# davenza/PyBNesian

Hardware: AMD Instinct MI355X
Metric: KDE slogl M-samples/s (higher is better)
Workload: dtype f64; 1 GPU; C2: ProductKDE.slogl f64, N_train=1000000, N_test=100000 per GPU, d=8, normal-reference diagonal bandwidth; parallelism=test rows sharded over 1 GPU(s), training set replicated, ranks=1

## Files before the change

### pybnesian_amd/csrc/capi.hip

```cpp
#include <algorithm>
#include <cmath>
#include <cstdlib>
#include <cstring>
#include <memory>
#include <numeric>

#include "common.hpp"
#include "hostmath.hpp"
#include "kde_kernels.hpp"
#include "kde_model.hpp"
#include "kde_handle.hpp"
#include "stats_kernels.hpp"

namespace pbn {
static thread_local std::string g_last_error;
void set_last_error(const std::string& s) { g_last_error = s; }
std::recursive_mutex& api_mutex() {
    static std::recursive_mutex m;
    return m;
}
}

using namespace pbn;

extern "C" {

const char* pbn_last_error(void) { return g_last_error.c_str(); }
const char* pbn_version(void) { return "pbn_hip 0.1 (gfx950)"; }

int pbn_ctx_create(int device, pbn_ctx** out) {
    return guarded([&] {
        if (!out) throw invalid_error("pbn_ctx_create: out is null");
        int count = 0;
        HIP_CHECK(hipGetDeviceCount(&count));
        if (device < 0 || device >= count) throw device_error("pbn_ctx_create: no such HIP device");
        HIP_CHECK(hipSetDevice(device));
        auto ctx = std::make_unique<pbn_ctx>();
        ctx->device = device;
        HIP_CHECK(hipStreamCreateWithFlags(&ctx->stream, hipStreamNonBlocking));
        hipDeviceProp_t prop;
        HIP_CHECK(hipGetDeviceProperties(&prop, device));
        ctx->num_cus = prop.multiProcessorCount > 0 ? prop.multiProcessorCount : 256;
        *out = ctx.release();
    });
}

}

void pbn::ctx_release(pbn_ctx* ctx) {
    if (ctx->refs.fetch_sub(1, std::memory_order_acq_rel) != 1) return;
    PBN_API_LOCK;
    (void)hipSetDevice(ctx->device);
    (void)hipStreamSynchronize(ctx->stream);
    ctx->scratch_part.release();
    ctx->scratch_q.release();
    ctx->scratch_misc.release();
    ctx->scratch_red.release();
    (void)hipStreamDestroy(ctx->stream);
    for (auto& ln : ctx->parked)
        if (ln.stream) { (void)hipStreamSynchronize(ln.stream); (void)hipStreamDestroy(ln.stream); (void)hipEventDestroy(ln.fence); }
    delete ctx;
}

extern "C" {

void pbn_ctx_destroy(pbn_ctx* ctx) {
    if (ctx) pbn::ctx_release(ctx);
}

int pbn_ctx_sync(pbn_ctx* ctx) {
    return guarded(mu_of(ctx), [&] {
        HIP_CHECK(hipSetDevice(ctx->device));
        HIP_CHECK(hipStreamSynchronize(ctx->stream));
    });
}

void* pbn_ctx_stream(pbn_ctx* ctx) { return (void*)ctx->stream; }

static void drain_timers(pbn_ctx* ctx) {
    HIP_CHECK(hipStreamSynchronize(ctx->stream));
    for (auto& t : ctx->pending) {
        float ms = 0.f;
        if (hipEventElapsedTime(&ms, t.e0, t.e1) == hipSuccess) {
            ctx->kernel_ms[t.which] += ms;
            ctx->kernel_launches[t.which] += 1;
        }
        (void)hipEventDestroy(t.e0);
        (void)hipEventDestroy(t.e1);
    }
    ctx->pending.clear();
}

int pbn_ctx_set_profiling(pbn_ctx* ctx, int on) {
    return guarded(mu_of(ctx), [&] {
        if (!ctx) throw invalid_error("pbn_ctx_set_profiling: null context");
        HIP_CHECK(hipSetDevice(ctx->device));
        drain_timers(ctx);
        ctx->profiling = on == 1;
        ctx->timing = on == 2;
        for (int i = 0; i < PBN_NUM_KERNEL_CLASSES; ++i) { ctx->kernel_ms[i] = 0; ctx->kernel_launches[i] = 0; }
    });
}

int pbn_ctx_kernel_time(pbn_ctx* ctx, int kernel_class, double* total_ms, int64_t* launches) {
    return guarded(mu_of(ctx), [&] {
        if (!ctx || kernel_class < 0 || kernel_class >= PBN_NUM_KERNEL_CLASSES) throw invalid_error("pbn_ctx_kernel_time: bad argument");
        HIP_CHECK(hipSetDevice(ctx->device));
        drain_timers(ctx);
        if (total_ms) *total_ms = ctx->kernel_ms[kernel_class];
        if (launches) *launches = ctx->kernel_launches[kernel_class];
    });
}

// ... 295 lines not shown
            k->cA.alloc((size_t)m.ntiles * k->cdf_KS * 64 * sizeof(double));
            k->cN.alloc((size_t)m.ntiles * 16 * sizeof(double));
            k->cU.alloc((size_t)m.ntiles * 16 * sizeof(double));
            pbn::WidePackArgs wa{};
            fill_cdf_pack_wide(ctx, wa, *k, train, cols);
            wa.rows = nullptr; wa.row0 = row0; wa.n0 = n; wa.row1 = 0; wa.n = n; wa.ntiles = m.ntiles; wa.is_query = 0;
            wa.pack = (double*)k->cA.p; wa.npack = (double*)k->cN.p; wa.upack = (double*)k->cU.p;
            KernelTimer kt(ctx, PBN_K_PACK);
            launch_pack_wide(wa, ctx->stream);
        }
    }
    *out = k.release();
}

int pbn_kde_fit(pbn_ctx* ctx, const pbn_table* train, const int* cols, int d, int64_t row0, int64_t n,
                const double* bandwidth, int kind, const double* center, pbn_kde** out) {
    return guarded(mu_of(ctx), [&] {
        if (kind != PBN_BW_FULL && kind != PBN_BW_DIAG) throw invalid_error("pbn_kde_fit: unknown bandwidth kind");
        kde_fit_impl(ctx, train, cols, d, row0, n, bandwidth, kind, false, center, out);
    });
}

int pbn_ckde_fit(pbn_ctx* ctx, const pbn_table* train, const int* cols, int d, int64_t row0, int64_t n,
                 const double* H, const double* center, pbn_kde** out) {
    return guarded(mu_of(ctx), [&] { kde_fit_impl(ctx, train, cols, d, row0, n, H, PBN_BW_FULL, true, center, out, true); });
}

void pbn_kde_destroy(pbn_kde* k) {
    if (!k) return;
    pbn::ctx_pin pin_(k->ctx);
    std::lock_guard<std::recursive_mutex> lock_(mu_of(k));
    (void)hipSetDevice(k->ctx->device);
    (void)hipStreamSynchronize(k->ctx->stream);
    delete k;
}

int64_t pbn_kde_num_instances(const pbn_kde* k) { return k ? k->m.N : 0; }
double pbn_kde_lognorm(const pbn_kde* k, int which) { return which ? k->m.lognorm_marg : k->m.lognorm; }

static void kde_eval_enqueue(pbn_kde* k, const pbn_table* test, const int* cols, int64_t row0, int64_t n,
                             double* dev_logl, double* dev_sum, bool precise = false) {
    if (!k) throw invalid_error("KDE factor not fitted.");
    if (k->split_joint) {
        pbn_ctx* ctx = k->ctx;
        check_cols(test, cols, k->m.d, "pbn_kde_logl");
        const size_t per = dev_logl ? (size_t)std::max<int64_t>(n, 1) : 0;
        ctx->scratch_split.reserve(2 * per + 2);
        double* lj = dev_logl ? ctx->scratch_split.p : nullptr;
        double* lm = dev_logl ? ctx->scratch_split.p + per : nullptr;
        double* sj = dev_sum ? ctx->scratch_split.p + 2 * per : nullptr;
        double* sm = dev_sum ? sj + 1 : nullptr;
        const bool lanes = pbn::score_lanes() > 1 && !ctx->profiling;
        if (lanes) { ctx->ensure_lanes(1); ctx->lanes_wait_for_stream(1); }
        pbn::kde_eval_enqueue(ctx, k->split_joint->m, test, cols, row0, n, lj, sj, nullptr, nullptr, precise);
        {
            pbn::LaneSwitch lane(ctx, lanes ? 1 : 0);
            pbn::kde_eval_enqueue(ctx, k->split_marg->m, test, cols + 1, row0, n, lm, sm, nullptr, nullptr, precise);
        }
        if (lanes) ctx->stream_waits_for_lane(0);
        if (dev_logl) launch_diff(dev_logl, lj, lm, n, ctx->stream);
        if (dev_sum) launch_diff(dev_sum, sj, sm, 1, ctx->stream);
        return;
    }
    pbn::kde_eval_enqueue(k->ctx, k->m, test, cols, row0, n, dev_logl, dev_sum, nullptr, nullptr, precise);
}

int pbn_kde_logl_dev(pbn_kde* k, const pbn_table* test, const int* cols, int64_t row0, int64_t n, double* dev_out) {
    return guarded(mu_of(k), [&] {
        if (!dev_out && n > 0) throw invalid_error("pbn_kde_logl_dev: null output");
        kde_eval_enqueue(k, test, cols, row0, n, dev_out, nullptr);
    });
}

int pbn_kde_logl(pbn_kde* k, const pbn_table* test, const int* cols, int64_t row0, int64_t n, double* out) {
    return guarded(mu_of(k), [&] {
        if (!out && n > 0) throw invalid_error("pbn_kde_logl: null output");
        if (!k) throw invalid_error("KDE factor not fitted.");
        dev_buf<double> tmp((size_t)std::max<int64_t>(n, 1));
        kde_eval_enqueue(k, test, cols, row0, n, tmp.p, nullptr);
        if (n > 0) HIP_CHECK(hipMemcpyAsync(out, tmp.p, (size_t)n * sizeof(double), hipMemcpyDeviceToHost, k->ctx->stream));
        HIP_CHECK(hipStreamSynchronize(k->ctx->stream));
    });
}

int pbn_ckde_cdf(pbn_kde* k, const pbn_table* test, const int* cols, int64_t row0, int64_t n, double* out) {
    return guarded(mu_of(k), [&] {
        if (!k) throw invalid_error("CKDE factor not fitted.");
        if (!k->ckde) throw invalid_error("pbn_ckde_cdf: the handle was not created by pbn_ckde_fit");
        if (!out && n > 0) throw invalid_error("pbn_ckde_cdf: null output");
        pbn_ctx* ctx = k->ctx;
        const KdeModel& m = k->m;
        check_cols(test, cols, m.d, "pbn_ckde_cdf");
        check_range(test, row0, n, "pbn_ckde_cdf");
        if (test->dtype != m.dtype) throw invalid_error("Data type of training and test datasets is different.");
        if (test->ctx->device != ctx->device) throw invalid_error("pbn_ckde_cdf: test table lives on another device");
        HIP_CHECK(hipSetDevice(ctx->device));
        if (n == 0) return;
        const int fdt = k->cdf_wide ? PBN_F64 : m.dtype;
        const size_t es = dtype_size(fdt);
        const int64_t nqtiles = ceil_div(n, 16);
        const size_t b_b = (size_t)nqtiles * k->cdf_KS * 64 * es, n_b = (size_t)nqtiles * 16 * es;
        ctx->scratch_q.reserve(b_b + 2 * n_b + 256);
        char* q = ctx->scratch_q.p;
        struct { void* pack; void* npack; void* upack; } pa{q, q + b_b, q + b_b + n_b};
        if (k->cdf_wide) {
            pbn::WidePackArgs wq{};
            fill_cdf_pack_wide(ctx, wq, *k, test, cols);
            wq.rows = nullptr; wq.row0 = row0; wq.n0 = n; wq.row1 = 0; wq.n = n; wq.ntiles = nqtiles; wq.is_query = 1;
            wq.pack = (double*)pa.pack; wq.npack = (double*)pa.npack; wq.upack = (double*)pa.upack;
            KernelTimer kt(ctx, PBN_K_PACK);
            launch_pack_wide(wq, ctx->stream);
        } else {
            PackArgs pq{};
            fill_cdf_pack(pq, *k, test, cols);
            pq.row0 = row0; pq.n0 = n; pq.row1 = 0; pq.n = n; pq.ntiles = nqtiles; pq.is_query = 1;
            pq.pack = pa.pack; pq.npack = pa.npack; pq.upack = pa.upack;
            KernelTimer kt(ctx, PBN_K_PACK);
// ... 47 lines not shown
```

### pybnesian_amd/csrc/common.hpp

```cpp
#pragma once
#include <hip/hip_runtime.h>
#include <cstdlib>
#include <utility>

#include <cstdarg>
#include <cstdint>
#include <cstdio>
#include <atomic>
#include <mutex>
#include <stdexcept>
#include <string>
#include <vector>

#include "../../include/pbn_hip.h"

#define PBN_MAX_D_HOST 33

namespace pbn {

struct invalid_error : std::runtime_error {
    using std::runtime_error::runtime_error;
};
struct singular_error : std::runtime_error {
    using std::runtime_error::runtime_error;
};
struct device_error : std::runtime_error {
    using std::runtime_error::runtime_error;
};

void set_last_error(const std::string& s);

std::recursive_mutex& api_mutex();
#define PBN_API_LOCK std::lock_guard<std::recursive_mutex> pbn_api_lock_(::pbn::api_mutex())

inline void hip_check(hipError_t e, const char* what, const char* file, int line) {
    if (e != hipSuccess) {
        char buf[512];
        snprintf(buf, sizeof buf, "HIP error %d (%s) in %s at %s:%d", (int)e, hipGetErrorString(e), what, file, line);
        throw device_error(buf);
    }
}
#define HIP_CHECK(x) ::pbn::hip_check((x), #x, __FILE__, __LINE__)

template <typename F>
int guarded(std::recursive_mutex& mu, F&& f) noexcept {
    try {
        std::lock_guard<std::recursive_mutex> lock(mu);
        f();
        return PBN_OK;
    } catch (const invalid_error& e) {
        set_last_error(e.what());
        return PBN_ERR_INVALID;
    } catch (const singular_error& e) {
        set_last_error(e.what());
        return PBN_ERR_SINGULAR;
    } catch (const device_error& e) {
        set_last_error(e.what());
        return PBN_ERR_DEVICE;
    } catch (const std::bad_alloc&) {
        set_last_error("out of host memory");
        return PBN_ERR_DEVICE;
    } catch (const std::exception& e) {
        set_last_error(e.what());
        return PBN_ERR_INVALID;
    }
}
template <typename F>
int guarded(F&& f) noexcept {
    return guarded(api_mutex(), std::forward<F>(f));
}

template <typename T>
struct dev_buf {
    T* p = nullptr;
    size_t n = 0;
    dev_buf() = default;
    explicit dev_buf(size_t count) { alloc(count); }
    dev_buf(const dev_buf&) = delete;
    dev_buf& operator=(const dev_buf&) = delete;
    dev_buf(dev_buf&& o) noexcept : p(o.p), n(o.n) { o.p = nullptr; o.n = 0; }
    dev_buf& operator=(dev_buf&& o) noexcept {
        if (this != &o) {
            release();
            p = o.p; n = o.n; o.p = nullptr; o.n = 0;
        }
        return *this;
    }
    ~dev_buf() { release(); }
    void alloc(size_t count) {
        release();
        n = count;
        if (count) HIP_CHECK(hipMalloc((void**)&p, count * sizeof(T)));
    }
    void reserve(size_t count) {
        if (count > n) alloc(count);
    }
    void release() {
        if (p) (void)hipFree(p);
        p = nullptr; n = 0;
    }
};

inline size_t dtype_size(int dtype) { return dtype == PBN_F32 ? 4 : 8; }

inline int64_t ceil_div(int64_t a, int64_t b) { return (a + b - 1) / b; }

}


struct pbn_ctx {
    std::recursive_mutex mu;
    std::atomic<int> refs{1};
    int device = 0;
    hipStream_t stream = nullptr;
    int num_cus = 256;
    pbn::dev_buf<char> scratch_part;
    pbn::dev_buf<char> scratch_q;
    pbn::dev_buf<char> scratch_misc;
    pbn::dev_buf<double> scratch_red;
    pbn::dev_buf<char> scratch_train;
    pbn::dev_buf<char> scratch_prune;
    pbn::dev_buf<char> scratch_pruneq;
    pbn::dev_buf<char> scratch_sort;
    pbn::dev_buf<double> scratch_split;
    pbn::dev_buf<double> scratch_w;
    pbn::dev_buf<char> scratch_group;
    pbn::dev_buf<double> scratch_sums;
    std::vector<std::vector<char>> staged;
    void drop_staged() { staged.clear(); }
    struct Lane {
        hipStream_t stream = nullptr;
        pbn::dev_buf<char> part, q, misc, train, prune, pruneq, sort, group;
        pbn::dev_buf<double> red, split, w;
        hipEvent_t fence = nullptr;
    };
    static constexpr int MAX_PARKED = 3;
    Lane parked[MAX_PARKED];
    void ensure_lanes(int n_parked) {
        for (int k = 0; k < n_parked && k < MAX_PARKED; ++k)
            if (!parked[k].stream) {
                HIP_CHECK(hipStreamCreateWithFlags(&parked[k].stream, hipStreamNonBlocking));
                HIP_CHECK(hipEventCreateWithFlags(&parked[k].fence, hipEventDisableTiming));
            }
    }
    void swap_lane(int k) {
        Lane& alt = parked[k];
        std::swap(stream, alt.stream);
        std::swap(scratch_part, alt.part); std::swap(scratch_q, alt.q); std::swap(scratch_misc, alt.misc);
        std::swap(scratch_train, alt.train); std::swap(scratch_prune, alt.prune); std::swap(scratch_pruneq, alt.pruneq);
        std::swap(scratch_sort, alt.sort); std::swap(scratch_group, alt.group); std::swap(scratch_red, alt.red); std::swap(scratch_split, alt.split); std::swap(scratch_w, alt.w);
    }
    void lanes_wait_for_stream(int n_parked) {
        for (int k = 0; k < n_parked && k < MAX_PARKED; ++k) {
            HIP_CHECK(hipEventRecord(parked[k].fence, stream));
            HIP_CHECK(hipStreamWaitEvent(parked[k].stream, parked[k].fence, 0));
        }
    }
    void stream_waits_for_lane(int k) {
        HIP_CHECK(hipEventRecord(parked[k].fence, parked[k].stream));
        HIP_CHECK(hipStreamWaitEvent(stream, parked[k].fence, 0));
    }
    void sync_lanes(int n_parked) {
        for (int k = 0; k < n_parked && k < MAX_PARKED; ++k)
            if (parked[k].stream) HIP_CHECK(hipStreamSynchronize(parked[k].stream));
    }
    bool profiling = false;
    bool timing = false;
    struct Timed { hipEvent_t e0, e1; int which; };
    std::vector<Timed> pending;
    double kernel_ms[PBN_NUM_KERNEL_CLASSES] = {0};
    int64_t kernel_launches[PBN_NUM_KERNEL_CLASSES] = {0};
};

namespace pbn {
void ctx_release(pbn_ctx* c);
inline void ctx_retain(pbn_ctx* c) { c->refs.fetch_add(1, std::memory_order_relaxed); }
struct ctx_ptr {
    pbn_ctx* p = nullptr;
    ctx_ptr() = default;
    ctx_ptr(const ctx_ptr&) = delete;
    ctx_ptr& operator=(const ctx_ptr&) = delete;
    ctx_ptr& operator=(pbn_ctx* c) {
        if (c) ctx_retain(c);
        if (p) ctx_release(p);
        p = c;
        return *this;
    }
    ~ctx_ptr() { if (p) ctx_release(p); }
    operator pbn_ctx*() const { return p; }
    pbn_ctx* operator->() const { return p; }
};
struct ctx_pin {
    pbn_ctx* c;
    explicit ctx_pin(pbn_ctx* c_) : c(c_) { if (c) ctx_retain(c); }
    ~ctx_pin() { if (c) ctx_release(c); }
    ctx_pin(const ctx_pin&) = delete;
    ctx_pin& operator=(const ctx_pin&) = delete;
};
}

namespace pbn {
inline std::recursive_mutex& mu_of(const pbn_ctx* c) { return c ? const_cast<pbn_ctx*>(c)->mu : api_mutex(); }
template <typename H>
inline std::recursive_mutex& mu_of(const H* h) { return h ? mu_of(static_cast<const pbn_ctx*>(h->ctx)) : api_mutex(); }
}

namespace pbn {
inline long long knob_ll(const char* name, long long dflt) { const char* e = std::getenv(name); return (e && *e) ? std::atoll(e) : dflt; }
inline int knob_int(const char* name, int dflt) { return (int)knob_ll(name, dflt); }
inline double knob_double(const char* name, double dflt) { const char* e = std::getenv(name); return (e && *e) ? std::atof(e) : dflt; }
}
#ifdef PBN_EXPERIMENTS
#define PBN_TUNE(NAME, dflt) (::pbn::knob_int("PBN_" #NAME, (int)(dflt)))
#define PBN_TUNE_D(NAME, dflt) (::pbn::knob_double("PBN_" #NAME, (double)(dflt)))
#else
#define PBN_TUNE(NAME, dflt) ((int)(dflt))
#define PBN_TUNE_D(NAME, dflt) ((double)(dflt))
#endif

namespace pbn {
inline int score_lanes(int64_t table_rows = -1) {
    static const int v = [] {
        const int n = knob_int("PBN_SCORE_LANES", 0);
        return n < 1 ? 0 : (n > 1 + pbn_ctx::MAX_PARKED ? 1 + pbn_ctx::MAX_PARKED : n);
    }();
    if (v) return v;
    return (table_rows >= 0 && table_rows <= 250000) ? 3 : 2;
}
struct LaneSwitch {
    pbn_ctx* ctx; int k;
    LaneSwitch(pbn_ctx* c, int lane) : ctx(c), k(lane - 1) { if (k >= 0) ctx->swap_lane(k); }
    ~LaneSwitch() { if (k >= 0) ctx->swap_lane(k); }
    LaneSwitch(const LaneSwitch&) = delete;
    LaneSwitch& operator=(const LaneSwitch&) = delete;
};
struct KernelTimer {
    pbn_ctx* ctx; int which; hipEvent_t e0 = nullptr;
    KernelTimer(pbn_ctx* c, int w) : ctx(c), which(w) {
        if (ctx->profiling || (ctx->timing && (w == PBN_K_SWEEP || w == PBN_K_GRAM || w == PBN_K_MOMENT))) { HIP_CHECK(hipEventCreate(&e0)); HIP_CHECK(hipEventRecord(e0, ctx->stream)); }
    }
    ~KernelTimer() {
        if (e0) {
            hipEvent_t e1;
            if (hipEventCreate(&e1) == hipSuccess && hipEventRecord(e1, ctx->stream) == hipSuccess)
                ctx->pending.push_back({e0, e1, which});
        }
    }
};
}

struct pbn_table {
    pbn::ctx_ptr ctx;
    int dtype = PBN_F64;
    int n_cols = 0;
    int64_t n_rows = 0;
    int64_t ld = 0;
    void* data = nullptr;
// ... 4 lines not shown
```

### pybnesian_amd/csrc/kde_model.hip

```cpp
#include <cstdio>
#include <algorithm>
#include <atomic>
#include <cmath>
#include <cstdlib>
#include <cstring>
#include <mutex>
#include <numeric>
#include <vector>

#include "hostmath.hpp"
#include "kde_kernels.hpp"
#include "kde_model.hpp"
#include "stats_kernels.hpp"

namespace pbn {

static const double LOG2E = 1.4426950408889634073599246810019;
static const double LOG_2PI = 1.8378770664093454835606594728112;

void check_cols(const pbn_table* t, const int* cols, int d, const char* who) {
    if (!t || !cols) throw invalid_error(std::string(who) + ": null argument");
    for (int i = 0; i < d; ++i)
        if (cols[i] < 0 || cols[i] >= t->n_cols) throw invalid_error(std::string(who) + ": column index out of range");
}
// ... 430 lines not shown
}

void kde_prune_persist(pbn_ctx* ctx, KdeModel& m, dev_buf<char>& store) {
    if (!m.prune) return;
    auto al = [](size_t x) { return (x + 255) / 256 * 256; };
    const size_t box_b = al((size_t)m.ntiles * 2 * m.pdims * sizeof(double)), zs_b = al((size_t)m.N * m.zdims * sizeof(double)),
                 key_b = al((size_t)m.N * sizeof(uint32_t));
    const SubBytes sb = sub_bytes(m, m.nsub);
    const bool screen = m.wfull && !m.cond && m.dm == 8 && m.zdims == 8 && m.pdims == PBN_PRUNE_PD && m.fdtype() == PBN_F64 && knob_int("PBN_D8_SCREEN", 1) != 0;
    const size_t sub_b = m.nsub ? al(sb.total) : 0, scr_b = screen ? al((size_t)m.ntiles * 16 * 32) : 0;
    const size_t plain_b = screen ? al((size_t)(ceil_div(m.ntiles, 64) + 1) * sizeof(unsigned long long)) : 0;
    const size_t fpack_b = screen ? al((size_t)m.ntiles * 768) : 0;
    store.alloc(box_b + zs_b + key_b + sub_b + scr_b + plain_b + fpack_b);
    HIP_CHECK(hipMemcpyAsync(store.p, m.tile_box, box_b, hipMemcpyDeviceToDevice, ctx->stream));
    HIP_CHECK(hipMemcpyAsync(store.p + box_b, m.zsorted, (size_t)m.N * m.zdims * sizeof(double), hipMemcpyDeviceToDevice, ctx->stream));
    HIP_CHECK(hipMemcpyAsync(store.p + box_b + zs_b, m.keys_sorted, (size_t)m.N * sizeof(uint32_t), hipMemcpyDeviceToDevice, ctx->stream));
    m.tile_box = (const double*)store.p;
    m.zsorted = (const double*)(store.p + box_b);
    m.keys_sorted = (const uint32_t*)(store.p + box_b + zs_b);
    if (m.nsub) {
        char* sp = store.p + box_b + zs_b + key_b;
        HIP_CHECK(hipMemcpyAsync(sp, m.Asub, sb.total, hipMemcpyDeviceToDevice, ctx->stream));
        m.Asub = sp; m.nxsub = sp + sb.a; m.Axsub = m.cond ? sp + sb.a + sb.n : nullptr;
    }
    m.scr = nullptr;
    if (screen) {
        char* sp = store.p + box_b + zs_b + key_b + sub_b;
        KernelTimer kt(ctx, PBN_K_PACK);
        launch_screen_pack(m.zsorted, nullptr, m.N, m.ntiles, false, sp, ctx->stream);
        m.scr = sp;
        launch_far_plain((const double*)m.nxpack, m.ntiles, (unsigned long long*)(sp + scr_b), ctx->stream);
        m.far_plain = (const unsigned long long*)(sp + scr_b);
        launch_far_pack(m.Apack, m.nxpack, m.ntiles, sp + scr_b + plain_b, ctx->stream);
        m.far_pack = sp + scr_b + plain_b;
    }
}

static std::atomic<bool> g_masks_capture{false};
static std::mutex g_masks_mu;
struct MaskDump {
    std::vector<unsigned long long> box, live, far;
    std::vector<double> qthr, zq, zt;
    std::vector<double> qrow;
    std::vector<double> part;
    long long dims[6] = {0, 0, 0, 0, 0, 0};
};
static MaskDump g_masks;

static std::atomic<bool> g_window_capture{false};
static std::mutex g_window_mu;
static std::vector<double> g_window_lb;
static std::vector<int64_t> g_window_pos;

void kde_eval_enqueue(pbn_ctx* ctx, const KdeModel& m, const pbn_table* test, const int* cols, int64_t row0, int64_t n,
                      double* dev_logl, double* dev_sum, const int32_t* dev_rows, double* dev_sum_marg, bool precise) {
    check_cols(test, cols, m.d, "pbn_kde_logl");
    const bool sum_only = dev_logl == nullptr && !precise;
    if (!dev_rows) check_range(test, row0, n, "pbn_kde_logl");
    if (test->dtype != m.dtype) throw invalid_error("Data type of training and test datasets is different.");
    const int fdt = m.fdtype();
    if (m.wide) {
        if (m.cond) throw invalid_error("KDE: a conditional model of more than 32 evidence variables is evaluated as joint - marginal");
        HIP_CHECK(hipSetDevice(ctx->device));
        if (n == 0) {
            if (dev_sum) HIP_CHECK(hipMemsetAsync(dev_sum, 0, sizeof(double), ctx->stream));
            return;
        }
        const int64_t nqt = ceil_div(n, 16);
        const size_t bp = (size_t)nqt * m.KS * 64 * sizeof(double), nyb = (size_t)nqt * 16 * sizeof(double);
        ctx->scratch_q.reserve(bp + nyb + 256);
        WidePackArgs wq{};
        fill_wide_pack(ctx, wq, test, cols, m);
        wq.rows = dev_rows; wq.row0 = row0; wq.n0 = n; wq.row1 = 0; wq.n = n; wq.ntiles = nqt; wq.is_query = 1;
        wq.pack = (double*)ctx->scratch_q.p; wq.npack = (double*)(ctx->scratch_q.p + bp);
        { KernelTimer kt(ctx, PBN_K_PACK); launch_pack_wide(wq, ctx->stream); }
        int64_t ns = std::max<int64_t>(1, ceil_div((int64_t)ctx->num_cus * 8, ceil_div(nqt, 4)));
        ns = std::min<int64_t>(ns, std::max<int64_t>(1, m.ntiles / 16));
        ns = std::min<int64_t>(ns, 1024);
        const int64_t tpsw = ceil_div(m.ntiles, ns);
        ns = ceil_div(m.ntiles, tpsw);
        ctx->scratch_part.reserve((size_t)ns * nqt * 16 * 2 * sizeof(double));
        SweepArgs sw{};
        sw.Apack = m.Apack; sw.nxpack = m.nxpack; sw.Bpack = wq.pack; sw.nypack = wq.npack;
        sw.ntiles = m.ntiles; sw.nqtiles = nqt; sw.tiles_per_split = tpsw; sw.part = (double*)ctx->scratch_part.p;
        { KernelTimer kt(ctx, PBN_K_SWEEP); launch_sweep_wide(sw, m.KS, (int)ns, ctx->stream); }
        const int64_t nb = ceil_div(n, 256);
        ctx->scratch_misc.reserve((size_t)nb * 2 * sizeof(double));
        FinishArgs fw{};
        fw.part = sw.part; fw.nsplit = (int)ns; fw.nqtiles = nqt; fw.nq = n;
        fw.lognorm = m.lognorm; fw.lognorm_marg = m.lognorm_marg;
        fw.logl = dev_logl; fw.scatter = nullptr; fw.block_sums = dev_sum ? (double*)ctx->scratch_misc.p : nullptr;
        { KernelTimer kt(ctx, PBN_K_FINISH); launch_finish(fw, false, dev_sum, ctx->stream, nullptr); }
        return;
    }
    if (test->ctx->device != ctx->device) throw invalid_error("pbn_kde_logl: test table lives on another device");
    HIP_CHECK(hipSetDevice(ctx->device));
    if (n == 0) {
        if (dev_sum) HIP_CHECK(hipMemsetAsync(dev_sum, 0, sizeof(double), ctx->stream));
        if (dev_sum_marg) HIP_CHECK(hipMemsetAsync(dev_sum_marg, 0, sizeof(double), ctx->stream));
        return;
    }
    const size_t es = dtype_size(fdt);
    const int64_t nqtiles = ceil_div(n, 16);
    const bool b3 = use_f16x2(fdt);
    const size_t bpack_b = b3 ? (size_t)nqtiles * m.KS * 64 * 16 : (size_t)nqtiles * m.KS * 64 * es,
                 ny_b = (size_t)nqtiles * 16 * es,
                 bx_b = m.cond ? (b3 ? (size_t)nqtiles * 64 * 16 : (size_t)nqtiles * 64 * es) : 0,
                 xn_b = (m.cond && b3) ? (size_t)nqtiles * 16 * 4 : 0,
                 ff_b = b3 ? ((size_t)nqtiles * 16 + 255) / 256 * 256 : 0;
    ctx->scratch_q.reserve(bpack_b + ny_b + bx_b + xn_b + ff_b + 512);
    char* q = ctx->scratch_q.p;
    PackArgs pa{};
    fill_pack_common(ctx, pa, test, cols, m);
    pa.rows = dev_rows;
    pa.row0 = row0; pa.n0 = n; pa.row1 = 0; pa.n = n; pa.ntiles = nqtiles;
    pa.is_query = 1;
    const bool fold = sweep_folds_norm(fdt, m.cond, m.KS, m.dm);
    pa.fold_norm = fold ? 1 : 0;
    const double* qbox = nullptr;
    const double* qthr = nullptr;
    const double* qlb = nullptr;
    const int32_t* qperm = nullptr;
    PruneSide qs{};
    const bool prune = m.prune && (sum_only || !m.wfull);
    const int window = (prune && m.wfull && m.KS == 2) ? std::max(0, knob_int("PBN_SUM_WINDOW", 256)) : 0;
    const bool wdbg = window > 0 && g_window_capture.load();
    const bool sdbg = prune && g_stages_capture.load();
    StageEval sev;
    int64_t* qtpos = nullptr;
    double* qdbg = nullptr;
    double* qrow = nullptr;
    double* qwpart = nullptr;
    const int wparts = window ? window_parts(nqtiles, ctx->num_cus) : 0;
    if (prune) {
        auto al = [](size_t x) { return (x + 255) / 256 * 256; };
        const size_t qbox_b = al((size_t)nqtiles * 2 * m.pdims * sizeof(double)), qthr_b = al((size_t)nqtiles * sizeof(double));
        const size_t qlb_b = al((size_t)nqtiles * 16 * sizeof(double));
        const size_t qtpos_b = (window || sdbg) ? al((size_t)nqtiles * sizeof(int64_t)) : 0, qdbg_b = wdbg ? al((size_t)nqtiles * 16 * sizeof(double)) : 0;
        const size_t qrow_b = window ? qlb_b : 0, qwpart_b = window ? al(window_part_bytes(nqtiles, wparts)) : 0;
        qs = prune_sort_side(ctx, ctx->scratch_pruneq, pa, fdt, m.zdims, m.kdims, qbox_b + qthr_b + qlb_b + qtpos_b + qdbg_b + qrow_b + qwpart_b);
        pa.perm = qs.perm;
        qperm = qs.perm;
        qbox = (double*)qs.rest; qthr = (double*)(qs.rest + qbox_b);
        static const bool use_qlb = PBN_TUNE(SWEEP_QLB, 1) != 0;
        if (use_qlb) qlb = (double*)(qs.rest + qbox_b + qthr_b);
        if (window || sdbg) qtpos = (int64_t*)(qs.rest + qbox_b + qthr_b + qlb_b);
        if (wdbg) qdbg = (double*)(qs.rest + qbox_b + qthr_b + qlb_b + qtpos_b);
        if (window) qrow = (double*)(qs.rest + qbox_b + qthr_b + qlb_b + qtpos_b + qdbg_b);
        if (window) qwpart = (double*)(qs.rest + qbox_b + qthr_b + qlb_b + qtpos_b + qdbg_b + qrow_b);
    }
    pa.pack = q; pa.npack = q + bpack_b; pa.xpack = m.cond ? q + bpack_b + ny_b : nullptr;
    pa.xnorm = xn_b ? q + bpack_b + ny_b + bx_b : nullptr;
    pa.far_flag = ff_b ? (unsigned char*)(q + ((bpack_b + ny_b + bx_b + xn_b + 255) / 256) * 256) : nullptr;
    { KernelTimer kt(ctx, PBN_K_PACK); launch_pack(pa, fdt, ctx->stream); }
    const int P = m.cond ? 4 : 2;
    const bool wmul = !fold && sweep_weights_norm(fdt, m.cond, m.KS, m.dm);
    if (prune) {
        const double* subpart = nullptr;
        if (m.nsub) {
            ctx->scratch_part.reserve((size_t)nqtiles * 16 * P * sizeof(double));
            SweepArgs ss{};
            ss.Apack = m.Asub; ss.nxpack = m.nxsub; ss.Axpack = m.Axsub;
            ss.Bpack = pa.pack; ss.nypack = pa.npack; ss.Bxpack = pa.xpack; ss.Bxnorm = pa.xnorm;
            ss.ntiles = m.ntiles_sub; ss.nqtiles = nqtiles; ss.tiles_per_split = m.ntiles_sub;
            ss.fold = fold ? 1 : 0; ss.wmul = wmul ? 1 : 0; ss.prune = 0;
            ss.part = (double*)ctx->scratch_part.p;
            { KernelTimer kt(ctx, PBN_K_PACK); launch_sweep(ss, fdt, m.KS, m.cond, 1, ctx->stream); }
            subpart = ss.part;
        }
        launch_query_prepass(qs.zrow, qs.perm, n, qs.keys, m.zsorted, m.keys_sorted, m.N, m.zdims, m.pdims, (double*)qbox, (double*)qthr, (double*)qlb,
                             ctx->stream, subpart, P, m.cond ? 2 : 0, subpart ? std::log2((double)m.nsub) : 0.0, m.cond ? nullptr : m.tile_box, qtpos, fdt);
        if (sdbg) {
            stage_fetch(sev.zrow, qs.zrow, (size_t)n * m.zdims, ctx->stream);
            stage_fetch(sev.keys_unsorted, qs.keys_unsorted, (size_t)n, ctx->stream);
            stage_fetch(sev.keys, qs.keys, (size_t)n, ctx->stream);
            stage_fetch(sev.qperm, qs.perm, (size_t)n, ctx->stream);
            stage_fetch(sev.subpart, subpart, subpart ? (size_t)nqtiles * 16 * P : 0, ctx->stream);
            stage_fetch(sev.qbox, qbox, (size_t)nqtiles * 2 * m.pdims, ctx->stream);
            stage_fetch(sev.qthr, qthr, (size_t)nqtiles, ctx->stream);
            stage_fetch(sev.qlb, qlb, qlb ? (size_t)nqtiles * 16 : 0, ctx->stream);
            stage_fetch(sev.qtpos, qtpos, (size_t)nqtiles, ctx->stream);
            HIP_CHECK(hipStreamSynchronize(ctx->stream));
            sev.num[1] = subpart ? std::log2((double)m.nsub) : 0.0;
        }
        if (window) {
            { KernelTimer kt(ctx, PBN_K_PACK); launch_query_window((const double*)m.Apack, (const double*)m.nxpack, (const double*)pa.pack, (const double*)pa.npack,
                                                               m.ntiles, m.N, nqtiles, n, qtpos, window, fold, (double*)qthr, (double*)qlb, qrow, qdbg, wparts, qwpart, ctx->stream); }
            if (wdbg) {
                std::vector<double> lb((size_t)n);
                std::vector<int32_t> perm((size_t)n);
                std::vector<int64_t> tpos((size_t)nqtiles);
                HIP_CHECK(hipMemcpyAsync(lb.data(), qdbg, (size_t)n * sizeof(double), hipMemcpyDeviceToHost, ctx->stream));
                HIP_CHECK(hipMemcpyAsync(tpos.data(), qtpos, (size_t)nqtiles * sizeof(int64_t), hipMemcpyDeviceToHost, ctx->stream));
                HIP_CHECK(hipMemcpyAsync(perm.data(), qperm, (size_t)n * sizeof(int32_t), hipMemcpyDeviceToHost, ctx->stream));
                HIP_CHECK(hipStreamSynchronize(ctx->stream));
                std::lock_guard<std::mutex> lk(g_window_mu);
                g_window_lb.assign((size_t)n, -INFINITY);
                for (int64_t i = 0; i < n; ++i) g_window_lb[(size_t)perm[(size_t)i]] = lb[(size_t)i];
                g_window_pos.assign((size_t)n, -1);
                for (int64_t i = 0; i < n; ++i) g_window_pos[(size_t)perm[(size_t)i]] = tpos[(size_t)(i >> 4)];
            }
        }
    }

    const int64_t qblocks = ceil_div(nqtiles, 4 * sweep_qg(fdt, m.cond, m.KS, prune));
    const int64_t target = (int64_t)ctx->num_cus * PBN_TUNE(SWEEP_BLOCKS_PER_CU, 24);
    int64_t nsplit = std::max<int64_t>(1, ceil_div(target, qblocks));
    const int64_t tile_bytes = b3 ? (int64_t)m.KS * 64 * 16 + (m.cond ? 64 * 16 : 0)
                                  : ((int64_t)m.KS * 64 + 16 + (m.cond ? 64 : 0)) * (int64_t)es;
    nsplit = std::max<int64_t>(nsplit, ceil_div(m.ntiles * tile_bytes, (int64_t)PBN_TUNE(SWEEP_SPLIT_KB, 2048) * 1024));
    if (prune) nsplit = std::max<int64_t>(nsplit, ceil_div(m.ntiles, (int64_t)PBN_TUNE(PRUNE_MAX_TILES, 1024)));
    if (nsplit > 1) nsplit = ceil_div(nsplit, 8) * 8;
    nsplit = std::min<int64_t>(nsplit, std::max<int64_t>(1, m.ntiles / PBN_TUNE(SWEEP_MIN_TILES, 64)));
    nsplit = std::min<int64_t>(nsplit, 4096);
    const int64_t tps = ceil_div(m.ntiles, nsplit);
    nsplit = ceil_div(m.ntiles, tps);
    static const int gmasks = PBN_TUNE(PRUNE_GROUP_MASKS, 1);
    const bool bboxes = prune && gmasks && !m.cond && fdt == PBN_F64 && PBN_TUNE(GROUP_BATCH_BOXES, 1) != 0;
    const size_t part_b = ((size_t)nsplit * nqtiles * 16 * P * sizeof(double) + 255) / 256 * 256;
    const size_t bbox_b = bboxes ? ((size_t)nsplit * ceil_div(tps, 64) * 2 * m.pdims * sizeof(double) + 255) / 256 * 256 : 0;
    const bool mdbg = g_masks_capture.load();
    bool screen = prune && sum_only && m.scr != nullptr && bboxes && wmul && m.KS == 2 && m.pdims == PBN_PRUNE_PD && m.zdims == 8 && knob_int("PBN_D8_SCREEN", 1) != 0;
    const size_t scrq_b = screen ? (size_t)nqtiles * 16 * 32 : 0;
    size_t mask_b = screen ? (size_t)ceil_div(nqtiles, PBN_QG_PRUNE) * nsplit * ceil_div(tps, 64) * PBN_QG_PRUNE * sizeof(unsigned long long) : 0;
    if (screen && (double)mask_b * (mdbg ? 2.0 : 1.0) > (double)knob_int("PBN_D8_SCREEN_MAX_MB", 512) * 1048576.0) screen = false;
    if (!screen) mask_b = 0;
    const bool rowthr = screen && qrow != nullptr && knob_int("PBN_D8_SCREEN_ROWTHR", 1) != 0;
    const double ftheta = far32_theta(m.N);
    const bool far = rowthr && m.far_plain != nullptr && knob_int("PBN_D8_FAR32", 1) != 0 && ftheta >= 8.0 && ftheta + 4.0 <= prune_margin(fdt, m.N, sum_only) &&
                     (double)mask_b * (mdbg ? 3.0 : 2.0) <= (double)knob_int("PBN_D8_SCREEN_MAX_MB", 512) * 1048576.0;
    const size_t part_rows_b = far ? ((size_t)2 * nsplit * nqtiles * 16 * P * sizeof(double) + 255) / 256 * 256 : part_b;
    ctx->scratch_part.reserve(part_rows_b + bbox_b + (screen ? scrq_b + mask_b * ((mdbg ? 2 : 1) + (far ? 1 : 0)) : 0));
    SweepArgs sa{};
    sa.Apack = m.Apack; sa.nxpack = m.nxpack; sa.Axpack = m.Axpack;
    sa.Bpack = pa.pack; sa.nypack = pa.npack; sa.Bxpack = pa.xpack; sa.Bxnorm = pa.xnorm;
    sa.ntiles = m.ntiles; sa.nqtiles = nqtiles; sa.tiles_per_split = tps;
    sa.fold = fold ? 1 : 0;
    sa.wmul = wmul ? 1 : 0;
    sa.w32 = (b3 && !m.cond && (prune ? f16x2_w32p(m.dm, m.KS) : f16x2_w32(m.dm, m.KS))) ? 1 : 0;
    sa.far_span = (sum_only && prune) ? (double)knob_int("PBN_FAR_SPAN", 17) : 0.0;
    const bool guard = knob_int("PBN_MAGIC_GUARD", 1) != 0;
    sa.tile_r = (guard && m.tile_r && !prune && sum_only) ? (const double*)((const char*)m.nxpack + (size_t)m.ntiles * 16 * es * 2) : nullptr;
    sa.fast = sum_only ? 1 : 0;
    sa.count_redo = knob_int("PBN_SWEEP_COUNT_REDO", 0);
    sa.box_full = (guard && prune && m.pdims == m.dm) ? 1 : 0;
    sa.prune = prune ? 1 : 0; sa.pdims = m.pdims; sa.prune_margin = prune_margin(fdt, m.N, sum_only); sa.tile_box = m.tile_box; sa.qtile_box = qbox; sa.qtile_thr = qthr; sa.qlb = qlb;
    sa.part = (double*)ctx->scratch_part.p;
    sa.group_masks = gmasks;
    if (bboxes) {
        double* bb = (double*)((char*)ctx->scratch_part.p + part_rows_b);
        launch_batch_boxes(m.tile_box, m.pdims, m.ntiles, tps, (int)nsplit, bb, ctx->stream);
        sa.batch_box = bb; sa.batches_per_split = (int)ceil_div(tps, 64);
    }
    static const bool log_sweeps = PBN_TUNE(SWEEP_LOG, 0) != 0;
    if (log_sweeps) std::fprintf(stderr, "pbn-sweep N=%lld n=%lld d=%d cond=%d prune=%d nsub=%lld nsplit=%lld\n", (long long)m.N, (long long)n, m.d, (int)m.cond, (int)prune, (long long)(prune ? m.nsub : 0), (long long)nsplit);
    if (screen) {
        char* sp = (char*)ctx->scratch_part.p + part_rows_b + bbox_b;
        sa.scr_train = m.scr; sa.scr_query = sp;
        sa.live_mask = (unsigned long long*)(sp + scrq_b);
        sa.box_mask = mdbg ? (unsigned long long*)(sp + scrq_b + mask_b) : nullptr;
        sa.qrow_thr = rowthr ? qrow : nullptr;
        if (far) {
            sa.far_mask = (unsigned long long*)(sp + scrq_b + mask_b * (mdbg ? 2 : 1));
            sa.tile_plain = m.far_plain;
            sa.far_theta = ftheta;
            sa.far_pack = m.far_pack;
        }
        KernelTimer kt(ctx, PBN_K_PACK);
        launch_screen_pack(qs.zrow, qs.perm, n, nqtiles, true, sp, ctx->stream);
        launch_screen_d8(sa, (int)nsplit, knob_int("PBN_D8_SCREEN_STREAM", 2), ctx->stream);
    }
    {
        KernelTimer kt(ctx, PBN_K_SWEEP);
        launch_sweep(sa, fdt, m.KS, m.cond, (int)nsplit, ctx->stream);
// ... 10 lines not shown
        HIP_CHECK(hipMemcpyAsync(g_masks.part.data(), sa.part, g_masks.part.size() * sizeof(double), hipMemcpyDeviceToHost, ctx->stream));
        std::vector<int32_t> perm((size_t)n);
        std::vector<double> zrow((size_t)n * 8);
        HIP_CHECK(hipMemcpyAsync(g_masks.box.data(), sa.box_mask, mask_b, hipMemcpyDeviceToHost, ctx->stream));
        HIP_CHECK(hipMemcpyAsync(g_masks.live.data(), sa.live_mask, mask_b, hipMemcpyDeviceToHost, ctx->stream));
        HIP_CHECK(hipMemcpyAsync(g_masks.qthr.data(), qthr, (size_t)nqtiles * sizeof(double), hipMemcpyDeviceToHost, ctx->stream));
        g_masks.qrow.resize((size_t)nqtiles * 16);
        if (sa.qrow_thr) HIP_CHECK(hipMemcpyAsync(g_masks.qrow.data(), sa.qrow_thr, (size_t)nqtiles * 16 * sizeof(double), hipMemcpyDeviceToHost, ctx->stream));
        HIP_CHECK(hipMemcpyAsync(zrow.data(), qs.zrow, (size_t)n * 8 * sizeof(double), hipMemcpyDeviceToHost, ctx->stream));
        HIP_CHECK(hipMemcpyAsync(perm.data(), qs.perm, (size_t)n * sizeof(int32_t), hipMemcpyDeviceToHost, ctx->stream));
        HIP_CHECK(hipStreamSynchronize(ctx->stream));
        for (int64_t i = 0; i < n; ++i)
            for (int k = 0; k < 8; ++k) g_masks.zq[(size_t)i * 8 + k] = zrow[(size_t)perm[(size_t)i] * 8 + k];
        for (auto& v : g_masks.qthr) v -= sa.prune_margin;
        if (sa.qrow_thr) {
            for (int64_t t = 0; t < nqtiles; ++t) {
                double top = g_masks.qrow[(size_t)t * 16] - sa.prune_margin;
                for (int c = 0; c < 16; ++c) {
                    double& v = g_masks.qrow[(size_t)t * 16 + c];
                    v -= sa.prune_margin;
                    if (v > top) top = v;
                }
                g_masks.qthr[(size_t)t] = top;
            }
        } else {
            for (int64_t t = 0; t < nqtiles; ++t)
                for (int c = 0; c < 16; ++c) g_masks.qrow[(size_t)t * 16 + c] = g_masks.qthr[(size_t)t];
        }
        const long long dims[6] = {(long long)ceil_div(nqtiles, PBN_QG_PRUNE), (long long)nsplit, (long long)ceil_div(tps, 64), (long long)tps, (long long)m.ntiles, (long long)n};
        for (int i = 0; i < 6; ++i) g_masks.dims[i] = dims[i];
    }
    if (b3) launch_far_fix(pa, m.Apack, m.Axpack, m.KS, m.N, m.ntiles, sa.part, (int)nsplit, nqtiles, m.cond, ctx->stream);

    if (sdbg) {
        const long long rows = sa.far_mask ? 2 * nsplit : nsplit;
        stage_fetch(sev.part, sa.part, (size_t)rows * nqtiles * 16 * P, ctx->stream);
        stage_fetch(sev.bbox, sa.batch_box, bboxes ? (size_t)nsplit * ceil_div(tps, 64) * 2 * m.pdims : 0, ctx->stream);
        HIP_CHECK(hipStreamSynchronize(ctx->stream));
        const long long head[21] = {(long long)n, (long long)nqtiles, (long long)nsplit, (long long)tps, (long long)ceil_div(tps, 64), sum_only ? 1 : 0, bboxes ? 1 : 0,
                                    qlb ? 1 : 0, window, m.nsub ? 1 : 0, P, m.cond ? 2 : 0, (long long)m.N, m.d, m.cond ? 1 : 0, fdt, rows,
                                    sweep_qg(fdt, m.cond, m.KS, true), ctx->num_cus, (long long)tile_bytes, m.KS};
        for (int i = 0; i < 21; ++i) sev.head[i] = head[i];
        sev.num[0] = sa.prune_margin;
        stage_keep(g_stage_evals, std::move(sev));
    }
    const int64_t nblocks = ceil_div(n, 256);
    ctx->scratch_misc.reserve((size_t)nblocks * 2 * sizeof(double));
    FinishArgs fa{};
    fa.part = sa.part; fa.nsplit = (int)(sa.far_mask ? 2 * nsplit : nsplit); fa.nqtiles = nqtiles; fa.nq = n;
    fa.lognorm = m.lognorm; fa.lognorm_marg = m.lognorm_marg;
    fa.logl = dev_logl; fa.scatter = qperm; fa.block_sums = dev_sum ? (double*)ctx->scratch_misc.p : nullptr;
    fa.block_sums_marg = (m.cond && dev_sum && dev_sum_marg) ? (double*)ctx->scratch_misc.p + nblocks : nullptr;
    { KernelTimer kt(ctx, PBN_K_FINISH); launch_finish(fa, m.cond, dev_sum, ctx->stream, dev_sum_marg); }
}

}

extern "C" int64_t pbn_debug_d8_masks(int what, void* out, int64_t cap, int capture) {
    pbn::g_masks_capture.store(capture != 0);
    std::lock_guard<std::mutex> lk(pbn::g_masks_mu);
    const pbn::MaskDump& d = pbn::g_masks;
    auto copy = [&](const void* src, size_t count, size_t size) -> int64_t {
        if (out && count) std::memcpy(out, src, std::min<size_t>(count, (size_t)std::max<int64_t>(cap, 0)) * size);
        return (int64_t)count;
    };
    switch (what) {
        case 0: return copy(d.dims, 6, sizeof(long long));
        case 1: return copy(d.box.data(), d.box.size(), 8);
        case 2: return copy(d.live.data(), d.live.size(), 8);
        case 3: return copy(d.qthr.data(), d.qthr.size(), 8);
        case 4: return copy(d.zq.data(), d.zq.size(), 8);
        case 5: return copy(d.zt.data(), d.zt.size(), 8);
        case 6: return copy(d.qrow.data(), d.qrow.size(), 8);
        case 7: return copy(d.far.data(), d.far.size(), 8);
        case 8: return copy(d.part.data(), d.part.size(), 8);
        default: return -1;
    }
}

extern "C" int64_t pbn_debug_sum_window(double* out, int64_t cap, int capture) {
    pbn::g_window_capture.store(capture != 0);
    std::lock_guard<std::mutex> lk(pbn::g_window_mu);
    const int64_t n = (int64_t)pbn::g_window_lb.size();
    for (int64_t i = 0; out && i < n && i < cap; ++i) out[i] = pbn::g_window_lb[(size_t)i];
    if (!capture) { pbn::g_window_lb.clear(); pbn::g_window_pos.clear(); }
    return n;
}

extern "C" int64_t pbn_debug_window_pos(int64_t* out, int64_t cap) {
    std::lock_guard<std::mutex> lk(pbn::g_window_mu);
    const int64_t n = (int64_t)pbn::g_window_pos.size();
    for (int64_t i = 0; out && i < n && i < cap; ++i) out[i] = pbn::g_window_pos[(size_t)i];
    return n;
}

extern "C" int64_t pbn_debug_prune_stages(int side, int back, int what, void* out, int64_t cap, int capture) {
    if (capture >= 0) pbn::g_stages_capture.store(capture != 0);
    std::lock_guard<std::mutex> lk(pbn::g_stages_mu);
    if (capture == 0) { pbn::g_stage_fits.clear(); pbn::g_stage_evals.clear(); }
    auto copy = [&](const void* src, size_t count, size_t size) -> int64_t {
        if (out && count) std::memcpy(out, src, std::min<size_t>(count, (size_t)std::max<int64_t>(cap, 0)) * size);
        return (int64_t)count;
    };
    if (side == 0) {
        const auto& all = pbn::g_stage_fits;
        if (what == -1) return (int64_t)all.size();
        if (back < 0 || (size_t)back >= all.size()) return -1;
        const pbn::StageFit& f = all[all.size() - 1 - (size_t)back];
        switch (what) {
            case 0: return copy(f.head, 14, 8);
            case 1: return copy(&f.cell, 1, 8);
            case 2: return copy(f.W.data(), f.W.size(), 8);
            case 3: return copy(f.mu.data(), f.mu.size(), 8);
            case 4: return copy(f.zrow.data(), f.zrow.size(), 8);
            case 5: return copy(f.keys_unsorted.data(), f.keys_unsorted.size(), 4);
            case 6: return copy(f.keys.data(), f.keys.size(), 4);
            case 7: return copy(f.perm.data(), f.perm.size(), 4);
            case 8: return copy(f.zsorted.data(), f.zsorted.size(), 8);
            case 9: return copy(f.box.data(), f.box.size(), 8);
            default: return -1;
        }
    }
    if (side == 1) {
        const auto& all = pbn::g_stage_evals;
        if (what == -1) return (int64_t)all.size();
        if (back < 0 || (size_t)back >= all.size()) return -1;
        const pbn::StageEval& e = all[all.size() - 1 - (size_t)back];
        switch (what) {
            case 0: return copy(e.head, 21, 8);
            case 1: return copy(e.num, 2, 8);
// ... 17 lines not shown
```

### pybnesian_amd/csrc/kde_model.hpp

```cpp
#pragma once
#include <cmath>
#include <vector>

#include "common.hpp"
#include "kde_kernels.hpp"

namespace pbn {

struct KdeModel {
    int dtype = PBN_F64;
    bool widen = false;
    int fdtype() const { return widen ? PBN_F64 : dtype; }
    int d = 0;
    int dm = 0;
    int KS = 0;
    bool cond = false;
    int64_t N = 0;
    int64_t ntiles = 0;
    double lognorm = 0.0, lognorm_marg = 0.0;
    std::vector<int> perm;
    bool wide = false;
    std::vector<double> W, mu;
    void* Apack = nullptr;
    void* nxpack = nullptr;
    bool tile_r = false;
    void* Axpack = nullptr;
    bool prune = false;
    int pdims = 0, zdims = 0;
    int kdims = 0;
    bool wfull = false;
    std::vector<double> Wrot;
    const double* tile_box = nullptr;
    const double* zsorted = nullptr;
    const uint32_t* keys_sorted = nullptr;
    int64_t nsub = 0, ntiles_sub = 0;
    void* Asub = nullptr;
    void* nxsub = nullptr;
    void* Axsub = nullptr;
    const void* scr = nullptr;
    const unsigned long long* far_plain = nullptr;
    const void* far_pack = nullptr;
};

struct KdePackBytes { size_t apack, nxpack, axpack; };
KdePackBytes kde_pack_bytes(int dtype, int dm, bool cond, int64_t n);

void kde_prepare(KdeModel& m, int dtype, int d, int64_t n, const double* bw, int kind, bool cond, const double* center);

double kde_max_norm2(pbn_ctx* ctx, const KdeModel& m, const pbn_table* t, const int* cols, int64_t row0, int64_t n0, int64_t row1,
                     const int32_t* dev_rows = nullptr);
bool kde_wants_widening(double max_norm2, int dm);
void kde_widen(KdeModel& m);

void kde_wide_pack_args(pbn_ctx* ctx, WidePackArgs& wa, const pbn_table* t, const int* cols_whitened, int d, int dm, const double* W, int ldw,
                        const double* mu, const double* wu);

void kde_pack_train(pbn_ctx* ctx, KdeModel& m, const pbn_table* t, const int* cols, int64_t row0, int64_t n0,
                    int64_t row1, const int32_t* dev_rows = nullptr, bool prune = false, double* dev_max_norm2 = nullptr);
bool kde_prune_applies(int dtype, int dm, int64_t n);
bool kde_prune_rotates(const KdeModel& m);
void kde_prune_persist(pbn_ctx* ctx, KdeModel& m, dev_buf<char>& store);

void kde_eval_enqueue(pbn_ctx* ctx, const KdeModel& m, const pbn_table* test, const int* cols, int64_t row0, int64_t n,
                      double* dev_logl, double* dev_sum, const int32_t* dev_rows = nullptr, double* dev_sum_marg = nullptr, bool precise = false);
inline bool kde_sum_needs_precision(double sum, int64_t n) { return n > 0 && std::fabs(sum) < PBN_TUNE_D(NEAR_ZERO_LOGL, 0.33) * (double)n; }

void bandwidth_from_cov(int selector, int kind, const double* cov, int d, int64_t n, int dtype, double* out);
void bandwidth_full_block(int selector, const double* cov, int d, int rule_d, int64_t n, int dtype, double* out);

void check_cols(const pbn_table* t, const int* cols, int d, const char* who);
void check_range(const pbn_table* t, int64_t row0, int64_t n, const char* who);

}
```

Measured before the change: 7.337 M-samples/s.

## Pipeline KDE query preprocessing on double-buffered front streams across calls

```diff
diff --git a/pybnesian_amd/csrc/capi.hip b/pybnesian_amd/csrc/capi.hip
--- a/pybnesian_amd/csrc/capi.hip
+++ b/pybnesian_amd/csrc/capi.hip
@@ -15,8 +15,8 @@
 namespace pbn {
 static thread_local std::string g_last_error;
 void set_last_error(const std::string& s) { g_last_error = s; }
-std::recursive_mutex& api_mutex() {
-    static std::recursive_mutex m;
+entry_mutex& api_mutex() {
+    static entry_mutex m;
     return m;
 }
 }
@@ -59,6 +59,9 @@
     (void)hipStreamDestroy(ctx->stream);
     for (auto& ln : ctx->parked)
         if (ln.stream) { (void)hipStreamSynchronize(ln.stream); (void)hipStreamDestroy(ln.stream); (void)hipEventDestroy(ln.fence); }
+    for (auto& f : ctx->front)
+        if (f.stream) { (void)hipStreamSynchronize(f.stream); (void)hipStreamDestroy(f.stream); (void)hipEventDestroy(f.ready); (void)hipEventDestroy(f.released); }
+    if (ctx->front_fence) (void)hipEventDestroy(ctx->front_fence);
     delete ctx;
 }
 
@@ -460,17 +463,17 @@
         double* sm = dev_sum ? sj + 1 : nullptr;
         const bool lanes = pbn::score_lanes() > 1 && !ctx->profiling;
         if (lanes) { ctx->ensure_lanes(1); ctx->lanes_wait_for_stream(1); }
-        pbn::kde_eval_enqueue(ctx, k->split_joint->m, test, cols, row0, n, lj, sj, nullptr, nullptr, precise);
+        pbn::kde_eval_enqueue(ctx, k->split_joint->m, test, cols, row0, n, lj, sj, nullptr, nullptr, precise, true);
         {
             pbn::LaneSwitch lane(ctx, lanes ? 1 : 0);
-            pbn::kde_eval_enqueue(ctx, k->split_marg->m, test, cols + 1, row0, n, lm, sm, nullptr, nullptr, precise);
+            pbn::kde_eval_enqueue(ctx, k->split_marg->m, test, cols + 1, row0, n, lm, sm, nullptr, nullptr, precise, true);
         }
         if (lanes) ctx->stream_waits_for_lane(0);
         if (dev_logl) launch_diff(dev_logl, lj, lm, n, ctx->stream);
         if (dev_sum) launch_diff(dev_sum, sj, sm, 1, ctx->stream);
         return;
     }
-    pbn::kde_eval_enqueue(k->ctx, k->m, test, cols, row0, n, dev_logl, dev_sum, nullptr, nullptr, precise);
+    pbn::kde_eval_enqueue(k->ctx, k->m, test, cols, row0, n, dev_logl, dev_sum, nullptr, nullptr, precise, true);
 }
 
 int pbn_kde_logl_dev(pbn_kde* k, const pbn_table* test, const int* cols, int64_t row0, int64_t n, double* dev_out) {
diff --git a/pybnesian_amd/csrc/common.hpp b/pybnesian_amd/csrc/common.hpp
--- a/pybnesian_amd/csrc/common.hpp
+++ b/pybnesian_amd/csrc/common.hpp
@@ -30,7 +30,11 @@
 
 void set_last_error(const std::string& s);
 
-std::recursive_mutex& api_mutex();
+struct entry_mutex : std::recursive_mutex {
+    uint64_t entries = 0;
+    int depth = 0;
+};
+entry_mutex& api_mutex();
 #define PBN_API_LOCK std::lock_guard<std::recursive_mutex> pbn_api_lock_(::pbn::api_mutex())
 
 inline void hip_check(hipError_t e, const char* what, const char* file, int line) {
@@ -66,6 +70,17 @@
     }
 }
 template <typename F>
+int guarded(entry_mutex& mu, F&& f) noexcept {
+    return guarded(static_cast<std::recursive_mutex&>(mu), [&] {
+        struct Scope {
+            entry_mutex& m;
+            explicit Scope(entry_mutex& m_) : m(m_) { ++m.entries; ++m.depth; }
+            ~Scope() { --m.depth; }
+        } scope(mu);
+        f();
+    });
+}
+template <typename F>
 int guarded(F&& f) noexcept {
     return guarded(api_mutex(), std::forward<F>(f));
 }
@@ -109,7 +124,7 @@
 
 
 struct pbn_ctx {
-    std::recursive_mutex mu;
+    pbn::entry_mutex mu;
     std::atomic<int> refs{1};
     int device = 0;
     hipStream_t stream = nullptr;
@@ -164,6 +179,32 @@
         for (int k = 0; k < n_parked && k < MAX_PARKED; ++k)
             if (parked[k].stream) HIP_CHECK(hipStreamSynchronize(parked[k].stream));
     }
+    struct Front {
+        hipStream_t stream = nullptr;
+        pbn::dev_buf<char> q, pruneq, sort, part;
+        hipEvent_t ready = nullptr, released = nullptr;
+        bool was_released = false;
+    };
+    Front front[2];
+    hipEvent_t front_fence = nullptr;
+    int front_next = 0;
+    int front_last = -1;
+    uint64_t front_exit = 0;
+    bool front_exit_valid = false;
+    void ensure_front() {
+        for (Front& f : front)
+            if (!f.stream) {
+                HIP_CHECK(hipStreamCreateWithFlags(&f.stream, hipStreamNonBlocking));
+                HIP_CHECK(hipEventCreateWithFlags(&f.ready, hipEventDisableTiming));
+                HIP_CHECK(hipEventCreateWithFlags(&f.released, hipEventDisableTiming));
+            }
+        if (!front_fence) HIP_CHECK(hipEventCreateWithFlags(&front_fence, hipEventDisableTiming));
+    }
+    void swap_front(int k) {
+        Front& f = front[k];
+        std::swap(stream, f.stream);
+        std::swap(scratch_q, f.q); std::swap(scratch_pruneq, f.pruneq); std::swap(scratch_sort, f.sort); std::swap(scratch_part, f.part);
+    }
     bool profiling = false;
     bool timing = false;
     struct Timed { hipEvent_t e0, e1; int which; };
@@ -200,9 +241,9 @@
 }
 
 namespace pbn {
-inline std::recursive_mutex& mu_of(const pbn_ctx* c) { return c ? const_cast<pbn_ctx*>(c)->mu : api_mutex(); }
+inline entry_mutex& mu_of(const pbn_ctx* c) { return c ? const_cast<pbn_ctx*>(c)->mu : api_mutex(); }
 template <typename H>
-inline std::recursive_mutex& mu_of(const H* h) { return h ? mu_of(static_cast<const pbn_ctx*>(h->ctx)) : api_mutex(); }
+inline entry_mutex& mu_of(const H* h) { return h ? mu_of(static_cast<const pbn_ctx*>(h->ctx)) : api_mutex(); }
 }
 
 namespace pbn {
diff --git a/pybnesian_amd/csrc/kde_model.hip b/pybnesian_amd/csrc/kde_model.hip
--- a/pybnesian_amd/csrc/kde_model.hip
+++ b/pybnesian_amd/csrc/kde_model.hip
@@ -506,8 +506,60 @@
 static std::vector<double> g_window_lb;
 static std::vector<int64_t> g_window_pos;
 
+static std::atomic<unsigned long long> g_front_evals{0}, g_front_chained{0};
+struct FrontStage {
+    pbn_ctx* ctx; int k = -1; bool open = false;
+    FrontStage(pbn_ctx* c, bool on) : ctx(c) {
+        if (!on) return;
+        ctx->ensure_front();
+        k = ctx->front_next;
+        ctx->front_next ^= 1;
+        pbn_ctx::Front& f = ctx->front[k];
+        if (f.was_released) HIP_CHECK(hipStreamWaitEvent(f.stream, f.released, 0));
+        const entry_mutex& mu = ctx->mu;
+        const bool chained = ctx->front_exit_valid && ctx->front_last >= 0 && mu.depth == 1 && (mu.entries == ctx->front_exit || mu.entries == ctx->front_exit + 1);
+        ctx->front_exit_valid = false;
+        if (chained) {
+            if (ctx->front_last != k) HIP_CHECK(hipStreamWaitEvent(f.stream, ctx->front[ctx->front_last].ready, 0));
+        } else {
+            HIP_CHECK(hipEventRecord(ctx->front_fence, ctx->stream));
+            HIP_CHECK(hipStreamWaitEvent(f.stream, ctx->front_fence, 0));
+        }
+        ctx->swap_front(k);
+        open = true;
+        g_front_evals.fetch_add(1);
+        if (chained) g_front_chained.fetch_add(1);
+    }
+    void join() {
+        if (!open) return;
+        open = false;
+        ctx->swap_front(k);
+        pbn_ctx::Front& f = ctx->front[k];
+        HIP_CHECK(hipEventRecord(f.ready, f.stream));
+        HIP_CHECK(hipStreamWaitEvent(ctx->stream, f.ready, 0));
+        ctx->front_last = k;
+    }
+    void release() {
+        if (k < 0) return;
+        pbn_ctx::Front& f = ctx->front[k];
+        HIP_CHECK(hipEventRecord(f.released, ctx->stream));
+        f.was_released = true;
+        ctx->front_exit = ctx->mu.entries;
+        ctx->front_exit_valid = ctx->mu.depth == 1;
+    }
+    ~FrontStage() {
+        if (!open) return;
+        ctx->swap_front(k);
+        pbn_ctx::Front& f = ctx->front[k];
+        if (hipEventRecord(f.ready, f.stream) == hipSuccess) { (void)hipStreamWaitEvent(ctx->stream, f.ready, 0); ctx->front_last = k; }
+        else (void)hipStreamSynchronize(f.stream);
+    }
+    FrontStage(const FrontStage&) = delete;
+    FrontStage& operator=(const FrontStage&) = delete;
+};
+
 void kde_eval_enqueue(pbn_ctx* ctx, const KdeModel& m, const pbn_table* test, const int* cols, int64_t row0, int64_t n,
-                      double* dev_logl, double* dev_sum, const int32_t* dev_rows, double* dev_sum_marg, bool precise) {
+                      double* dev_logl, double* dev_sum, const int32_t* dev_rows, double* dev_sum_marg, bool precise, bool front_lanes) {
     check_cols(test, cols, m.d, "pbn_kde_logl");
     const bool sum_only = dev_logl == nullptr && !precise;
     if (!dev_rows) check_range(test, row0, n, "pbn_kde_logl");
@@ -556,6 +608,9 @@
     }
     const size_t es = dtype_size(fdt);
     const int64_t nqtiles = ceil_div(n, 16);
+    const bool prune = m.prune && (sum_only || !m.wfull);
+    const bool cap_stages = g_stages_capture.load(), cap_window = g_window_capture.load(), cap_masks = g_masks_capture.load();
+    FrontStage front(ctx, front_lanes && prune && m.d <= PBN_W_INLINE_D && !cap_stages && !cap_window && !cap_masks && knob_int("PBN_KDE_PIPELINE", 1) != 0);
     const bool b3 = use_f16x2(fdt);
     const size_t bpack_b = b3 ? (size_t)nqtiles * m.KS * 64 * 16 : (size_t)nqtiles * m.KS * 64 * es,
                  ny_b = (size_t)nqtiles * 16 * es,
@@ -576,10 +631,9 @@
     const double* qlb = nullptr;
     const int32_t* qperm = nullptr;
     PruneSide qs{};
-    const bool prune = m.prune && (sum_only || !m.wfull);
     const int window = (prune && m.wfull && m.KS == 2) ? std::max(0, knob_int("PBN_SUM_WINDOW", 256)) : 0;
-    const bool wdbg = window > 0 && g_window_capture.load();
-    const bool sdbg = prune && g_stages_capture.load();
+    const bool wdbg = window > 0 && cap_window;
+    const bool sdbg = prune && cap_stages;
     StageEval sev;
     int64_t* qtpos = nullptr;
     double* qdbg = nullptr;
@@ -656,6 +710,7 @@
             }
         }
     }
+    front.join();
 
     const int64_t qblocks = ceil_div(nqtiles, 4 * sweep_qg(fdt, m.cond, m.KS, prune));
     const int64_t target = (int64_t)ctx->num_cus * PBN_TUNE(SWEEP_BLOCKS_PER_CU, 24);
@@ -673,7 +728,7 @@
     const bool bboxes = prune && gmasks && !m.cond && fdt == PBN_F64 && PBN_TUNE(GROUP_BATCH_BOXES, 1) != 0;
     const size_t part_b = ((size_t)nsplit * nqtiles * 16 * P * sizeof(double) + 255) / 256 * 256;
     const size_t bbox_b = bboxes ? ((size_t)nsplit * ceil_div(tps, 64) * 2 * m.pdims * sizeof(double) + 255) / 256 * 256 : 0;
-    const bool mdbg = g_masks_capture.load();
+    const bool mdbg = cap_masks;
     bool screen = prune && sum_only && m.scr != nullptr && bboxes && wmul && m.KS == 2 && m.pdims == PBN_PRUNE_PD && m.zdims == 8 && knob_int("PBN_D8_SCREEN", 1) != 0;
     const size_t scrq_b = screen ? (size_t)nqtiles * 16 * 32 : 0;
     size_t mask_b = screen ? (size_t)ceil_div(nqtiles, PBN_QG_PRUNE) * nsplit * ceil_div(tps, 64) * PBN_QG_PRUNE * sizeof(unsigned long long) : 0;
@@ -790,6 +845,7 @@
     fa.logl = dev_logl; fa.scatter = qperm; fa.block_sums = dev_sum ? (double*)ctx->scratch_misc.p : nullptr;
     fa.block_sums_marg = (m.cond && dev_sum && dev_sum_marg) ? (double*)ctx->scratch_misc.p + nblocks : nullptr;
     { KernelTimer kt(ctx, PBN_K_FINISH); launch_finish(fa, m.cond, dev_sum, ctx->stream, dev_sum_marg); }
+    front.release();
 }
 
 }
@@ -814,6 +870,12 @@
         case 8: return copy(d.part.data(), d.part.size(), 8);
         default: return -1;
     }
+}
+
+extern "C" void pbn_debug_front_lanes(unsigned long long* evals, unsigned long long* chained, int reset) {
+    if (evals) *evals = pbn::g_front_evals.load();
+    if (chained) *chained = pbn::g_front_chained.load();
+    if (reset) { pbn::g_front_evals.store(0); pbn::g_front_chained.store(0); }
 }
 
 extern "C" int64_t pbn_debug_sum_window(double* out, int64_t cap, int capture) {
diff --git a/pybnesian_amd/csrc/kde_model.hpp b/pybnesian_amd/csrc/kde_model.hpp
--- a/pybnesian_amd/csrc/kde_model.hpp
+++ b/pybnesian_amd/csrc/kde_model.hpp
@@ -62,7 +62,8 @@
 void kde_prune_persist(pbn_ctx* ctx, KdeModel& m, dev_buf<char>& store);
 
 void kde_eval_enqueue(pbn_ctx* ctx, const KdeModel& m, const pbn_table* test, const int* cols, int64_t row0, int64_t n,
-                      double* dev_logl, double* dev_sum, const int32_t* dev_rows = nullptr, double* dev_sum_marg = nullptr, bool precise = false);
+                      double* dev_logl, double* dev_sum, const int32_t* dev_rows = nullptr, double* dev_sum_marg = nullptr, bool precise = false,
+                      bool front_lanes = false);
 inline bool kde_sum_needs_precision(double sum, int64_t n) { return n > 0 && std::fabs(sum) < PBN_TUNE_D(NEAR_ZERO_LOGL, 0.33) * (double)n; }
 
 void bandwidth_from_cov(int selector, int kind, const double* cov, int d, int64_t n, int dtype, double* out);
```

Result: faster. 7.638 M-samples/s (median of 6 runs) (+4.1%).
